# sqlp/sedumi

Hardware: AMD Instinct MI355X
Metric: IPM iters/sec (ADA' form+factor+solve) (higher is better)
Workload: dtype f64; 1 GPU; control07.mat: examples/control07.mat (BASELINE.json configs[1]), m=666, nnz(At)=107940, nnz(ADA')=443556, nnz(L)=222111; unit = getada1+2+3, blkchol, 4x(fwblkslv,./d,bwblkslv); parallelism=single GPU

## Files before the change

include/sedumi_hip.h:

```cpp
#ifndef SEDUMI_HIP_H
#define SEDUMI_HIP_H

#include <stdint.h>

#ifdef __cplusplus
extern "C" {
#endif

typedef int64_t sdm_int;

const char *sdm_last_error(void);
const char *sdm_backend(void);
int sdm_device_count(void);
int sdm_set_device(int dev);

typedef struct {
  double canceltol;
  double maxu;
  double abstol;
} sdm_cholpars;

typedef struct {
  sdm_int lpN;
  sdm_int lorN;
// ... 156 lines not shown

int sdm_plan_set_dense(sdm_plan *p, sdm_int nden, const sdm_int *LADjc, const sdm_int *LADir, const sdm_int *dzjc,
                       const sdm_int *dzir, const sdm_int *colperm, const sdm_int *first);
int sdm_plan_deninfac(sdm_plan *p, const double *smult, double maxuden, int *host_fallback);
int sdm_plan_lden(sdm_plan *p, sdm_int *betajc, double *beta, double *pv, sdm_int *pivperm, sdm_int *npivperm,
                  sdm_int *dopiv, double *Ld);

int sdm_plan_set_growth_max(sdm_plan *p, double growth_max);
int sdm_plan_set_refinement(sdm_plan *p, int mode, double refine_max);
int sdm_plan_set_one_launch_fronts(sdm_plan *p, int on);
int sdm_plan_set_tile_workgroups(sdm_plan *p, int n);
int sdm_plan_set_one_launch_inverse(sdm_plan *p, int on);
int sdm_plan_set_solve_width(sdm_plan *p, sdm_int width);
int sdm_plan_get_solve_width(sdm_plan *p, sdm_int *width);
int sdm_plan_solve_stats(sdm_plan *p, sdm_int *nblocks, sdm_int *nbad, double *max_growth);

int sdm_plan_set_active_supernodes(sdm_plan *p, const int *active, sdm_int nsuper);
int sdm_plan_front_layout(sdm_plan *p, sdm_int *nlevels, sdm_int *level, sdm_int *foff, sdm_int *fsize, sdm_int *woff, sdm_int *ms, sdm_int *first, sdm_int *ns);
int sdm_plan_blkchol_begin(sdm_plan *p, const sdm_cholpars *pars, int use_absd);
int sdm_plan_blkchol_levels(sdm_plan *p, sdm_int l0, sdm_int l1, int extend_only);
int sdm_plan_blkchol_end(sdm_plan *p);
int sdm_plan_solve_levels(sdm_plan *p, int what, sdm_int l0, sdm_int l1);

int sdm_plan_blkchol_panels(sdm_plan *p, sdm_int l0, sdm_int l1, sdm_int pan0, sdm_int pan1, int world, int rank, int blk);
int sdm_plan_panel_record(sdm_plan *p, sdm_int panel, int unpack, sdm_int *front_offset, sdm_int *front_nelem);

int sdm_mexcache_getada1(sdm_int m, const sdm_int *ADAjc, const sdm_int *ADAir, sdm_int N, const sdm_int *Ajc, const sdm_int *Air,
                         const double *Apr, const sdm_int *Ajc2, const sdm_int *perm, sdm_int lpN, const double *dl, sdm_int lorN,
                         const double *ddet, const sdm_int *qblkstart, double *ADApr, double token_in, double *token_out);
int sdm_mexcache_getada2(sdm_int m, const sdm_int *ADAjc, const sdm_int *ADAir, const double *ADApr_in, double *ADApr, sdm_int lorN,
// ... 37 lines not shown
```

sedumi_amd/capi.py:

```python
from __future__ import annotations

import ctypes as C
import os

import numpy as np

_HERE = os.path.dirname(os.path.abspath(__file__))
DEFAULT_LIB = os.path.join(_HERE, "lib", "libsedumi_hip.so")
_lib = None
_lib_path = None

I64P = C.POINTER(C.c_int64)
F64P = C.POINTER(C.c_double)


class SdmError(RuntimeError):
    pass


class CholPars(C.Structure):
    _fields_ = [("canceltol", C.c_double), ("maxu", C.c_double), ("abstol", C.c_double)]


class CgPars(C.Structure):
# ... 24 lines not shown
                       "(hipcc, gfx950).  sedumi_amd has no CPU fallback.")
    L = C.CDLL(path)
    L.sdm_last_error.restype = C.c_char_p
    L.sdm_backend.restype = C.c_char_p
    L.sdm_plan_create.restype = C.c_void_p
    L.sdm_plan_create.argtypes = [C.c_int, C.c_void_p]
    L.sdm_plan_destroy.argtypes = [C.c_void_p]
    L.sdm_plan_devptr.restype = C.c_void_p
    L.sdm_plan_devptr.argtypes = [C.c_void_p, C.c_char_p, I64P]
    for name in ("sdm_plan_sync", "sdm_plan_getada", "sdm_plan_getdatq", "sdm_plan_fwsolve", "sdm_plan_bwsolve", "sdm_plan_ldlsolve"):
        getattr(L, name).argtypes = [C.c_void_p]
    L.sdm_plan_blkchol.argtypes = [C.c_void_p, C.POINTER(CholPars), C.c_int]
    L.sdm_plan_upload.argtypes = [C.c_void_p, C.c_char_p, F64P, C.c_int64]
    L.sdm_plan_download.argtypes = [C.c_void_p, C.c_char_p, F64P, C.c_int64]
    L.sdm_plan_wrappcg.argtypes = [C.c_void_p, C.POINTER(CgPars), C.c_double, C.c_int, C.c_int, I64P, I64P]
    L.sdm_plan_timer_begin.argtypes = [C.c_void_p, C.c_int]
    L.sdm_plan_timer_end.argtypes = [C.c_void_p, C.c_int]
    L.sdm_plan_timer_ms.argtypes = [C.c_void_p, C.c_int, C.POINTER(C.c_float)]
    _lib = L
    return L


def check(rc):
    if rc:
        raise SdmError(lib().sdm_last_error().decode())


def backend():
    return lib().sdm_backend().decode()

# ... 27 lines not shown
```

sedumi_amd/csrc/sdm_ada.hip:

```cpp
#include "sdm_plan.h"
#include <algorithm>
#include <cmath>
#include <cstdlib>

namespace sdm {

__global__ void k_dsqr(double *dsqr, const int *code, const double *dl, const double *ddet, int nlq) {
  int r = blockIdx.x * blockDim.x + threadIdx.x;
  if (r < nlq) { int c = code[r]; dsqr[r] = c == -1 ? dl[r] : (c >= 0 ? ddet[c] : -ddet[-2 - c]); }
}
__global__ void k_fill(double *x, double v, int64_t n) {
  int64_t t = (int64_t)blockIdx.x * blockDim.x + threadIdx.x;
  int64_t stride = (int64_t)gridDim.x * blockDim.x;
  for (; t < n; t += stride) x[t] = v;
}

constexpr int SPDOT_CAP = 2048;
template <int LPE>
__global__ void __launch_bounds__(256)
k_ada_spdot(double *ada, const int64_t *ADAjc, const int *ADAir, const int64_t *Mbeg, const int64_t *Mend,
            const int *Mir, const double *Mpr, const double *wgt, const int *invperm, int accumulate, int jbase, int cap) {
  SDM_DYN_SMEM(smem);
  double *jv = (double *)smem;
  int *jr = (int *)(jv + cap);
// ... 654 lines not shown
        }
        const double term = Apr[p] * (zv / 2);
        acc += term; aabs += fabs(term);
      }
    const double base = base_zero ? 0.0 : ada[e];
    ada[e] = base + acc;
    if (i == j) absd[j] = jhas ? base + aabs : 0.0;
  }
}

template <int JB>
__global__ void __launch_bounds__(64 * ELL_WAVES)
k_psd_stage2_ell(double *ada, double *absd, const int64_t *ADAjc, const int *ADAir, const int64_t *Ajc,
                 const int64_t *Ajc_psd, const double *Apr, const int *Ablk, const int *Aupos,
                 const int64_t *c_taskptr, const int *t_blk, const int *t_ulen, const int64_t *t_zoff, const double *zbuf,
                 const int64_t *uoff, const int *g_row, const int *g_len, const int64_t *g_off, const double *g_val,
                 const int *g_pos, int ngroups, const int *invperm, int zmax, int m, int jbase, int jend, const int *ell_pos, const int *ell_order,
                 const int *Azpos, const int *t_zdst, int base_zero, const long long *cd64, const int *cd32) {
  SDM_DYN_SMEM(smem);
  double *zl = (double *)smem;
  __shared__ double absred[JB][ELL_WAVES];
  __shared__ double part[JB][ELL_WAVES][64];
  const int j0 = jbase + blockIdx.x * JB;
  const int tid = threadIdx.x, bs = blockDim.x;
  const int wave = tid >> 6, lane = tid & 63, nw = bs >> 6;
  int gq[JB], gstart = 0;
  if (ell_order) {
    gstart = ngroups;
#pragma unroll
    for (int q = 0; q < JB; q++) { gq[q] = min(j0 + q, jend - 1) >> 6; gstart = min(gstart, gq[q]); }
  } else {
#pragma unroll
    for (int q = 0; q < JB; q++) gq[q] = 0;
  }
  constexpr int SEG_MAX = 4 * JB;
  __shared__ long long sg_src[SEG_MAX];
  __shared__ int sg_dst[SEG_MAX], sg_cum[SEG_MAX + 1];
  __shared__ long long tb_s[JB], te_s[JB], ab_s[JB], ae_s[JB];
  __shared__ int jc_s[JB];
  for (int k = tid; k < zmax * JB; k += bs) zl[k] = 0.0;
  if (tid < SEG_MAX) {
    const int q = tid >> 2, sgi = tid & 3;
    const int x = min(j0 + q, jend - 1);
    const bool in = j0 + q < jend;
    const int nt = cd32[16 * x + 1];
    if (sgi == 0) {
      jc_s[q] = cd32[16 * x];
      const long long tb = cd64[8 * x];
      tb_s[q] = in ? tb : 0; te_s[q] = in ? tb + nt : 0;
      ab_s[q] = in ? cd64[8 * x + 1] : 0; ae_s[q] = in ? cd64[8 * x + 2] : 0;
    }
    const bool live = in && sgi < nt;
    sg_src[tid] = cd64[8 * x + 3 + sgi]; sg_dst[tid] = q * zmax + cd32[16 * x + 2 + sgi]; sg_cum[tid + 1] = live ? cd32[16 * x + 6 + sgi] : 0;
  }
  if (tid == 0) sg_cum[0] = 0;
  const int g0 = gstart + (int)blockIdx.y;
  int i0 = -1, len0 = 0;
  long long off0 = 0;
  if (g0 < ngroups) { i0 = g_row[g0 * 64 + lane]; len0 = g_len[g0]; off0 = g_off[g0]; }
  __syncthreads();
#define ELLCOL(x) (jc_s[(x) - j0 < JB ? (x) - j0 : JB - 1])
  bool jhas[JB], own[JB], owns = false;
  bool inl = true;
#pragma unroll
  for (int q = 0; q < JB; q++) {
    jhas[q] = te_s[q] > tb_s[q];
    inl = inl && te_s[q] - tb_s[q] <= 4;
    const int grp = ell_order ? gq[q] : (ell_pos[min(j0 + q, jend - 1)] >> 6);
    own[q] = j0 + q < jend && (int)blockIdx.y == (grp - gstart) % (int)gridDim.y;
    owns = owns || own[q];
  }
  if (inl) {
    if (tid == 0) for (int x = 0; x < SEG_MAX; x++) sg_cum[x + 1] += sg_cum[x];
    __syncthreads();
    const int ntot = sg_cum[SEG_MAX];
    for (int base = 0; base < ntot; base += 12 * bs) {
      double v[12]; int dd[12];
#pragma unroll
      for (int x = 0; x < 12; x++) {
        const int idx = base + x * bs + tid;
        dd[x] = -1; v[x] = 0.0;
        if (idx < ntot) {
          int sgi = 0;
          while (idx >= sg_cum[sgi + 1]) sgi++;
// ... 30 lines not shown
    __syncthreads();
    if (tid < JB && own[tid]) {
      const int j = ELLCOL(j0 + tid);
      double basev = 0.0;
      int64_t lo = ADAjc[j], hi = ADAjc[j + 1];
      const int64_t ce = hi;
      if (ce - lo == m) lo += j;
      else while (lo < hi) { const int64_t mid = (lo + hi) >> 1; if (ADAir[mid] < j) lo = mid + 1; else hi = mid; }
      if (lo < ce && ADAir[lo] == j) basev = ada[lo];
      double a = 0.0;
      for (int w = 0; w < nw; w++) a += absred[tid][w];
      absd[j] = jhas[tid] ? basev + a : 0.0;
    }
    __syncthreads();
  }
  for (int g = g0; g < ngroups; g += gridDim.y) {
    const bool first = g == g0;
    const int i = first ? i0 : g_row[g * 64 + lane];
    const int len = first ? len0 : g_len[g];
    const int64_t goff = first ? off0 : g_off[g];
    const double *gv = g_val + goff * 64 + lane;
    const int *gp = g_pos + goff * 64 + lane;
    double acc[JB];
#pragma unroll
    for (int q = 0; q < JB; q++) acc[q] = 0.0;
    int t = wave;
    for (; t + 7 * nw < len; t += 8 * nw) {
      double v[8]; int pos[8];
#pragma unroll
      for (int x = 0; x < 8; x++) { const int64_t tt = t + x * nw; v[x] = gv[tt * 64]; pos[x] = gp[tt * 64]; }
#pragma unroll
      for (int x = 0; x < 8; x++)
#pragma unroll
        for (int q = 0; q < JB; q++) acc[q] += v[x] * zl[(size_t)q * zmax + pos[x]];
    }
// ... 104 lines not shown
  if (A.q_dense) {
    SDM_HIP_CHECK(hipMemsetAsync(A.Q_d.p, 0, (size_t)A.lorN * (size_t)A.m * sizeof(double), P->stream));
    SDM_KLAUNCH(P, k_q_densify, dim3((unsigned)((A.nnzQ + 255) / 256)), dim3(256), 0, A.Q_d.p, A.qpr.p, A.q_dst.p, (int64_t)A.nnzQ);
    launch_gram(P, ada, A.Q_d.p, nullptr, A.lorN, nullptr, 0, d_invperm, accumulate, nullptr);
  } else launch_spdot(P, ada, A.d_Qjc.p, A.d_Qjc.p + 1, A.d_Qir.p, A.qpr.p, nullptr, A.q_maxcol, d_invperm, accumulate);
}
bool ada_lq_q(sdm_plan *P, double *ada) {
  AdaPlan &A = P->ada;
  if (!(A.lq_dense && A.q_dense && A.q_src.n && A.col0 == 0 && A.col1 == A.m && A.lorN > 0 && A.nnzQ > 0)) return false;
  const int64_t nq = (int64_t)A.lorN * (int)A.m, nprep = std::max<int64_t>(nq, A.nlq);
  SDM_KLAUNCH(P, k_lq_q_prep, dim3((unsigned)((nprep + 255) / 256)), dim3(256), 0, A.dsqr.p, A.dsqr_code.p, A.dl.p, A.ddet.p, (int)A.nlq,
              A.Q_d.p, A.qpr.p, A.q_src.p, nq);
  launch_gram(P, ada, A.Alq_d.p, A.dsqr.p, A.nlq, A.Q_d.p, A.lorN, nullptr, false, A.sdpN == 0 ? P->absd.p : nullptr);
  return true;
}
static void symmetrize_in_place(sdm_plan *P, double *ada) {
  AdaPlan &A = P->ada;
  SDM_KLAUNCH(P, k_symmetrize, dim3((int)A.m), dim3(128), 0, A.symtmp.p, ada, A.d_ADAjc.p, A.d_ADAir.p, A.d_ADAT.p, (int)A.m);
  SDM_HIP_CHECK(hipMemcpyAsync(ada, A.symtmp.p, A.symtmp.n * sizeof(double), hipMemcpyDeviceToDevice, P->stream));
}
static Stage1Tab stage1_tab(const AdaPlan &A) {
  Stage1Tab T;
  T.t_n = A.t_n.p; T.t_nslot = A.t_nslot.p; T.t_ulen = A.t_ulen.p; T.t_herm = A.t_herm.p; T.s_col = A.s_col.p;
  T.u_pos = A.u_pos.p; T.u_rc = A.u_rc.p; T.Air = A.d_Air.p; T.t_slotptr = A.t_slotptr.p; T.t_udoff = A.t_udoff.p; T.t_uoff = A.t_uoff.p;
  T.t_zoff = A.t_zoff.p; T.t_end = A.t_end.p; T.s_nzptr = A.s_nzptr.p; T.Apr = A.d_Apr.p; T.t_blk = A.t_blk.p;
  T.psd_start = A.d_psd_start.p;
  return T;
}
static Stage2Ride stage2_ride(sdm_plan *P, double *ada, const int *d_invperm) {
  const AdaPlan &A = P->ada;
  Stage2Ride R2 = {};
  R2.ada = ada; R2.absd = P->absd.p; R2.ADAjc = A.d_ADAjc.p; R2.Ajc = A.d_Ajc.p; R2.Ajc_psd = A.d_Ajc_psd.p; R2.ADAir = A.d_ADAir.p;
  R2.Ablk = A.d_Ablk.p; R2.Aupos = A.d_Aupos.p; R2.t_col = A.t_col.p; R2.invperm = d_invperm; R2.Apr = A.d_Apr.p;
  return R2;
}
template <int JB>
static void launch_stage2_ell(sdm_plan *P, double *ada, const int *d_invperm, int ncols, int jbase, bool sym, int gsplit, bool cleared) {
  AdaPlan &A = P->ada;
  const size_t lds = (size_t)JB * (size_t)A.zmax * sizeof(double);
#ifndef SDM_EMU
  if (lds > 48 * 1024) SDM_HIP_CHECK(hipFuncSetAttribute((const void *)k_psd_stage2_ell<JB>, hipFuncAttributeMaxDynamicSharedMemorySize, (int)lds));
#endif
  SDM_KLAUNCH_AS(P, P->stream, JB == 4 ? "k_psd_stage2_ell<4>" : JB == 2 ? "k_psd_stage2_ell<2>" : "k_psd_stage2_ell<1>", k_psd_stage2_ell<JB>,
                 dim3((ncols + JB - 1) / JB, gsplit), dim3(64 * ELL_WAVES), lds, ada, P->absd.p, A.d_ADAjc.p, A.d_ADAir.p,
                 A.d_Ajc.p, A.d_Ajc_psd.p, A.d_Apr.p, A.d_Ablk.p, A.d_Aupos.p, A.c_taskptr.p, A.t_blk.p, A.t_ulen.p,
                 A.t_zoff.p, A.zbuf.p, A.d_uoff.p, A.g_row.p, A.g_len.p, A.g_off.p, A.g_val.p, A.g_bu.p, A.ell_ng, d_invperm,
                 (int)A.zmax, (int)A.m, jbase, jbase + ncols, A.ell_pos.p, sym ? (const int *)A.ell_order.p : (const int *)nullptr,
                 A.d_Azpos.p, A.t_zdst.p, cleared ? 1 : 0,
                 sym ? (const long long *)A.cdp64.p : (const long long *)A.cdc64.p, sym ? (const int *)A.cdp32.p : (const int *)A.cdc32.p);
}
void ada_psd(sdm_plan *P, double *ada, const int *d_invperm, bool sym_input, bool absd_done) {
  AdaPlan &A = P->ada;
  const int m = (int)A.m;
  if (A.sdpN == 0 || sym_input || A.col1 <= A.col0) ada_zero_flush(P);
  if (A.sdpN == 0) {
    if (sym_input) symmetrize_in_place(P, ada);
    if (!absd_done) SDM_KLAUNCH(P, k_diag, dim3((m + 255) / 256), dim3(256), 0, P->absd.p, ada, A.d_ADAjc.p, A.d_ADAir.p, m);
    return;
  }
  if (A.col1 <= A.col0) return;
  const int ncols = (int)(A.col1 - A.col0), jbase = (int)A.col0;
  const int task0 = (int)A.h_taskptr[A.col0], ntask = (int)(A.h_taskptr[A.col1] - A.h_taskptr[A.col0]);
  const size_t direct_lds = (size_t)(2 * A.sdpN + 2 * S1_DIRECT_MAXNZ * A.sdpN + 2) * sizeof(int) + (size_t)(2 * A.sdpN) * sizeof(long long) +
                            (size_t)(S1_DIRECT_MAXNZ * A.sdpN) * sizeof(double);
// ... 47 lines not shown
      const bool ride = A.one_task_per_col && A.thread_per_row && !A.ell_ok && A.sdpN == A.rsdpN && A.s1_maxulen <= 6 * 512 &&
                        (int64_t)A.s1_maxulen * (int64_t)sizeof(double) <= (int64_t)ldsy;
      if (ride) {
        if (sym_input) symmetrize_in_place(P, ada);
        SDM_HIP_CHECK(hipMemsetAsync(P->absd.p + jbase, 0, (size_t)ncols * sizeof(double), P->stream));
      }
      SDM_KLAUNCH(P, k_psd_stage1, dim3((unsigned)ntask), dim3(512), lds, T, A.udsqr.p, A.zbuf.p, (int)(ldsy / sizeof(double)), task0, nzcap,
                  ride ? stage2_ride(P, ada, d_invperm) : Stage2Ride{},
                  (ntask == (int)A.ntask && A.t_order_xcd.n == (size_t)ntask) ? (const int *)A.t_order_xcd.p : (const int *)nullptr);
      if (ride) { SDM_HIP_CHECK(hipGetLastError()); return; }
    }
  }
  if (sym_input) symmetrize_in_place(P, ada);
  if (A.ell_ok) {
    const bool sym = A.ell_full && !d_invperm && jbase == 0 && ncols == m;
    const int gsplit = sym ? 3 : 1;
    const bool cleared = stage1_cleared_all && !sym_input;
    const size_t zbytes = (size_t)A.zmax * sizeof(double);
    if (4 * zbytes <= 64 * 1024 && m >= 1024) launch_stage2_ell<4>(P, ada, d_invperm, ncols, jbase, sym, gsplit, cleared);
    else if (2 * zbytes <= 64 * 1024 && m >= 512) launch_stage2_ell<2>(P, ada, d_invperm, ncols, jbase, sym, gsplit, cleared);
    else launch_stage2_ell<1>(P, ada, d_invperm, ncols, jbase, sym, gsplit, cleared);
  } else {
    const int64_t zl = (A.thread_per_row && A.zmaxj * 8 <= 64 * 1024) ? A.zmaxj : 0;
    const size_t lds = (size_t)A.sdpN * 8 + (size_t)zl * 8;
#ifndef SDM_EMU
    if (lds > 48 * 1024) SDM_HIP_CHECK(hipFuncSetAttribute((const void *)k_psd_stage2, hipFuncAttributeMaxDynamicSharedMemorySize, (int)lds));
#endif
    SDM_KLAUNCH(P, k_psd_stage2, dim3(ncols), dim3(256), lds, ada, P->absd.p, A.d_ADAjc.p, A.d_ADAir.p, A.d_Ajc.p,
               A.d_Ajc_psd.p, A.d_Apr.p, A.d_Ablk.p, A.d_Aupos.p, A.c_taskptr.p, A.t_blk.p, A.t_zoff.p, A.c_zlen.p, A.zbuf.p,
               d_invperm, (int)A.sdpN, A.thread_per_row ? 1 : 0, jbase, (int)zl);
  }
  SDM_HIP_CHECK(hipGetLastError());
}

}

// ... 8 lines not shown
```

sedumi_amd/csrc/sdm_ada_build.hip:

```cpp
#include "sdm_plan.h"
#include <algorithm>

namespace sdm {
namespace {

struct AdaIn {
  sdm_int m; const sdm_int *Ajc, *Air; const double *Apr; const sdm_int *Ajc_psd;
  sdm_int lpN, lorN, sdpN, rsdpN; const sdm_int *sdpNL, *qblkstart, *psd_blkstart, *Qjc, *Qir, *ADAjc, *ADAir;
  sdm_int psd_begin(sdm_int j) const { return sdpN > 0 ? Ajc_psd[j] : Ajc[j + 1]; }
};
struct PsdPatterns {
  std::vector<int> Ablk, Aupos;
  std::vector<std::vector<int>> U;
  std::vector<int64_t> uoff;
  sdm_int psdnnz = 0;
};
struct Stage1Tasks {
  std::vector<int> t_col, t_blk, t_n, t_nslot, t_ulen, t_herm, s_col, order, order_xcd;
  std::vector<int64_t> t_slotptr, t_udoff, t_uoff, t_zoff, t_end, s_nzptr, c_taskptr, c_zlen;
};

void upload_narrow(DevBuf<int> &d, const sdm_int *h, sdm_int n) { std::vector<int> v((size_t)n); for (sdm_int t = 0; t < n; t++) v[t] = (int)h[t]; d.upload(v); }

PsdPatterns psd_patterns(AdaPlan &A, const AdaIn &in) {
// ... 138 lines not shown
  std::vector<int> zp((size_t)A.nnzA, 0);
  for (sdm_int i = 0; i < m; i++) for (sdm_int t = Ajc_psd[i]; t < Ajc[i + 1]; t++) zp[(size_t)t] = (int)(pt.uoff[pt.Ablk[t]] + pt.Aupos[t]);
  std::vector<int> zd(tk.t_blk.size());
  for (size_t t = 0; t < tk.t_blk.size(); t++) zd[t] = (int)pt.uoff[tk.t_blk[t]];
  std::vector<double> gval((size_t)goff[ng] * 64, 0.0);
  std::vector<int> gbu((size_t)goff[ng] * 64, 0);
  for (int g = 0; g < ng; g++)
    for (int l = 0; l < 64; l++) {
      const int i = grow[g * 64 + l];
      if (i < 0) continue;
      for (sdm_int t = Ajc_psd[i]; t < Ajc[i + 1]; t++) {
        const size_t pos = (size_t)(goff[g] + (t - Ajc_psd[i])) * 64 + l;
        gval[pos] = in.Apr[t]; gbu[pos] = zp[(size_t)t];
      }
    }
  A.ell_ng = ng;
  A.g_row.upload(grow); A.g_len.upload(glen); A.g_off.upload(goff); A.g_val.upload(gval); A.g_bu.upload(gbu);
  { std::vector<int> pos((size_t)m); for (sdm_int p = 0; p < m; p++) pos[(size_t)order[p]] = (int)p; A.ell_pos.upload(pos); }
  A.ell_order.upload(order);
  A.ell_full = (in.ADAjc[m] == (sdm_int)m * m);
  A.d_uoff.upload(pt.uoff); A.d_Azpos.upload(zp); A.t_zdst.upload(zd);
  ell_column_records(in, tk, zd, nullptr, A.cdc64, A.cdc32);
  ell_column_records(in, tk, zd, order.data(), A.cdp64, A.cdp32);
  A.ell_ok = true;
}

std::vector<int> ada_transpose_map(const AdaIn &in) {
  const sdm_int m = in.m, *ADAjc = in.ADAjc, *ADAir = in.ADAir;
  std::vector<int> adaT((size_t)ADAjc[m], -1);
  for (sdm_int j = 0; j < m; j++)
    for (sdm_int e = ADAjc[j]; e < ADAjc[j + 1]; e++) {
      sdm_int i = ADAir[e];
      const sdm_int *b = ADAir + ADAjc[i], *en = ADAir + ADAjc[i + 1];
      const sdm_int *f = std::lower_bound(b, en, j);
      if (f != en && *f == j) adaT[e] = (int)(f - ADAir);
    }
  return adaT;
}

void lq_dense_forms(AdaPlan &A, const AdaIn &in) {
// ... 82 lines not shown
  const AdaIn in = {m, Ajc, Air, Apr, Ajc_psd, lpN, lorN, sdpN, rsdpN, sdpNL, qblkstart, psd_blkstart, Qjc, Qir, ADAjc, ADAir};
  A.N = N; A.m = m; A.nnzA = Ajc[m]; A.lpN = lpN; A.lorN = lorN; A.sdpN = sdpN; A.rsdpN = rsdpN;
  A.ic_n.release(); A.ufac.release();
  if (A.nnzA >= (sdm_int)1 << 31 || N >= (sdm_int)1 << 31) throw std::runtime_error("At too large for 32-bit row indices");
  A.nlq = sdpN > 0 ? psd_blkstart[0] : N;
  if (lorN > 0 && qblkstart[lorN] != A.nlq && sdpN > 0) throw std::runtime_error("qblkstart / psd_blkstart mismatch");
  const PsdPatterns pt = psd_patterns(A, in);
  A.thread_per_row = (m > 0 && pt.psdnnz / (double)m < 48.0);
  A.nnz_lq = A.nnzA - pt.psdnnz;
  A.nnzQ = lorN > 0 ? Qjc[m] : 0;
  A.lq_maxcol = 0; A.q_maxcol = 0;
  for (sdm_int j = 0; j < m; j++) A.lq_maxcol = std::max<int64_t>(A.lq_maxcol, in.psd_begin(j) - Ajc[j]);
  for (sdm_int j = 0; j < m && lorN > 0; j++) A.q_maxcol = std::max<int64_t>(A.q_maxcol, Qjc[j + 1] - Qjc[j]);
  const Stage1Tasks tk = stage1_tasks(A, in, pt);
  stage2_ell(A, in, pt, tk);
  upload_tables(A, in, pt, tk, ada_transpose_map(in));
  lq_dense_forms(A, in);
  P->has_ada = true;
}

}
```

sedumi_amd/csrc/sdm_capi.hip:

```cpp
#include "../../include/sedumi_hip.h"
#include "sdm_plan.h"
#include <algorithm>
#include <cstring>
#include <memory>

namespace sdm {
static thread_local std::string g_err;
void set_error(const std::string &msg) { g_err = msg; }
}
using namespace sdm;

static const char *const FACTOR_TIMEOUT = "blkchol: a workgroup timed out waiting for another one inside a factor launch";
static void check_plan_health(sdm_plan *p) {
  const int t = chol_wait_timeouts(p);
  if (t & TMO_FACTOR) throw std::runtime_error(FACTOR_TIMEOUT);
  if (t & TMO_SWEEP) throw std::runtime_error("solve: a workgroup timed out waiting for another one inside a merged sweep launch (the factor stays; the next solves run unmerged)");
}
static sdm_cholpars chol_pars(const sdm_cholpars *pars) {
  sdm_cholpars q = {1e-12, 5e2, 1e-20};
  if (pars) q = *pars;
  if (q.abstol < 0.0) q.abstol = 0.0;
  return q;
}
static void require_begun(sdm_plan *p, const char *fn) {
// ... 365 lines not shown
  SDM_CATCH
}
int sdm_plan_set_solve_width(sdm_plan *p, sdm_int width) {
  SDM_TRY
  if (width != 0 && (width < sdm::SBW_MIN || width > sdm::SBW_MAX || (width & (width - 1)) != 0))
    throw std::runtime_error("solve width must be 0 (automatic) or a power of two in 256 .. 2048");
  p->chol.sbw_req = (int)width;
  SDM_CATCH
}
int sdm_plan_get_solve_width(sdm_plan *p, sdm_int *width) {
  SDM_TRY
  if (!p->has_chol) throw std::runtime_error("sdm_plan_get_solve_width: no symbolic factor set");
  *width = p->chol.sbw;
  SDM_CATCH
}
int sdm_plan_solve_stats(sdm_plan *p, sdm_int *nblocks, sdm_int *nbad, double *max_growth) {
  SDM_TRY
  if (!p->has_chol) throw std::runtime_error("sdm_plan_solve_stats: no symbolic factor set");
  solve_stats(p, nblocks, nbad, max_growth);
  SDM_CATCH
}
int sdm_plan_pcg_init(sdm_plan *p, sdm_int nden, const sdm_int *dense_cols, const double *denseA) {
  SDM_TRY
  if (!p->has_ada) throw std::runtime_error("sdm_plan_pcg_init: no problem data set (sdm_plan_set_ada)");
  SDM_HIP_CHECK(hipSetDevice(p->device));
  pcg_set_dense(p, nden, dense_cols, denseA);
  SDM_CATCH
}
int sdm_plan_amul(sdm_plan *p, int transp) {
  SDM_TRY
// ... 420 lines not shown
```

sedumi_amd/csrc/sdm_plan.h:

```cpp
#pragma once
#include "../../include/sedumi_hip.h"
#include "sdm_rt.h"
#include <mutex>
#include <string>
#include <vector>

namespace sdm {

constexpr int NB = 64;
constexpr int TILE = 64;
constexpr int UTP = 72;
constexpr int S1_MAXN = 96;
constexpr int S1_KC = 32;
constexpr int S1_WAVES = 8;
constexpr int S1_NZ = 1536;
constexpr int s1_nzcap(int64_t maxnz) { return (int)(((maxnz + 1) & ~(int64_t)1) < S1_NZ ? ((maxnz + 1) & ~(int64_t)1) : S1_NZ); }
constexpr int s1_mfma_ldsy(int maxn) { return 2 * S1_KC * ((maxn + 15) & ~15) > maxn * (maxn | 1) ? 2 * S1_KC * ((maxn + 15) & ~15) : maxn * (maxn | 1); }
constexpr size_t s1_mfma_lds(int maxn, int64_t maxnz) { return (size_t)s1_mfma_ldsy(maxn) * sizeof(double) + (size_t)s1_nzcap(maxnz) * (sizeof(double) + sizeof(int)); }
constexpr int S1_MAXT = ((S1_MAXN / 16) * (S1_MAXN / 16) + S1_WAVES - 1) / S1_WAVES;
constexpr int S1_GEN_LDS = 74 * 1024;
constexpr int ELL_WAVES = 8;
constexpr int SOLVE_LDS_MAX = 3072;
constexpr int FUSE_MAX_TILES = 1 << 20;
constexpr int SBW_MIN = 256;
// ... 178 lines not shown
  int sweep_seq = 0;
  HostFlag noted;
};

struct FrontTab {
  const int *first, *ns, *ms, *ld;
  const int64_t *foff, *xl, *woff, *roff, *toff;
  const int *childptr, *childlist, *lindx, *relidx;
  const int64_t *soff; const int *sld, *sboff;
  const int64_t *ltoff = nullptr;
  const int *fslot = nullptr;
  int one = 0, o_s = 0, o_ns = 0, o_ms = 0, o_ld = 0, o_first = 0, o_sld = 0, o_sboff = 0;
  int64_t o_foff = 0, o_soff = 0, o_woff = 0, o_xl = 0, o_ltoff = 0;
};

struct AdaPlan {
  sdm_int N = 0, m = 0, nnzA = 0, lpN = 0, lorN = 0, sdpN = 0, rsdpN = 0;
  sdm_int nlq = 0;
  sdm_int lenud = 0, ntask = 0, zlen = 0, nnzQ = 0, nnz_lq = 0;
  int maxn = 0;
  bool thread_per_row = false;
  sdm_int col0 = 0, col1 = 0;
  double *zero_ptr = nullptr; long long zero_n = 0; bool zero_defer = false;
  std::vector<int64_t> h_taskptr;
  std::vector<sdm_int> psd_n, psd_start, psd_udoff;
  DevBuf<int64_t> d_Ajc, d_Ajc_psd, d_Qjc, d_ADAjc;
  DevBuf<int> d_Air, d_Qir, d_ADAir, d_ADAT;
  DevBuf<double> d_Apr;
  DevBuf<int> d_Ablk, d_Aupos;
  DevBuf<int> t_col, t_blk, t_n, t_nslot, t_ulen, t_herm, t_order, t_order_xcd;
// ... 30 lines not shown
  PinnedInts wp_host;
  size_t stage1_lds = 0;
  bool ell_ok = false;
  int ell_ng = 0;
  int64_t zmax = 0, zmaxj = 0;
  DevBuf<int64_t> c_zlen;
  DevBuf<int> g_row, g_len, g_bu;
  DevBuf<long long> cdc64, cdp64;
  DevBuf<int> cdc32, cdp32;
  DevBuf<int> d_Azpos, t_zdst;
  DevBuf<int> ell_pos;
  DevBuf<int> ell_order;
  bool ell_full = false;
  DevBuf<int64_t> g_off, d_uoff;
  DevBuf<double> g_val;
};

}

namespace sdm {
struct KProf {
  bool enabled = false;
  struct Rec { const char *name; hipEvent_t a, b; };
  std::vector<Rec> recs;
  std::vector<hipEvent_t> pool;
  hipEvent_t get() {
    if (!pool.empty()) { hipEvent_t e = pool.back(); pool.pop_back(); return e; }
    hipEvent_t e; SDM_HIP_CHECK(hipEventCreate(&e)); return e;
  }
};
// ... 143 lines not shown
                      const double *Apr, const sdm_int *Ajc2, sdm_int lpN, sdm_int lorN, const sdm_int *qblkstart);
void gw_run_getada1(sdm_plan *p, const int *d_invperm, const double *dl, const double *ddet);
void gw_build_getada2(sdm_plan *p, sdm_int m, const sdm_int *ADAjc, const sdm_int *ADAir, sdm_int lorN, const sdm_int *Qjc, const sdm_int *Qir);
void gw_run_getada2(sdm_plan *p, const int *d_invperm, const double *Qpr);
void gw_build_getada3(sdm_plan *p, sdm_int m, const sdm_int *ADAjc, const sdm_int *ADAir, sdm_int N, const sdm_int *Ajc, const sdm_int *Air,
                      const double *Apr, const sdm_int *Ajc1, const sdm_cone *K, const sdm_int *psd_blkstart);
void gw_run_getada3(sdm_plan *p, const double *udsqr, bool input_is_zero);
bool gw_getada1_is_zero(sdm_plan *p);
void gw_build_getada(sdm_plan *p, sdm_int m, const sdm_int *ADAjc, const sdm_int *ADAir, const sdm_int *Ajc, const sdm_int *Air, const double *Apr,
                     sdm_int lpN, sdm_int lorN, const sdm_int *qblkstart, const sdm_int *Qjc, const sdm_int *Qir);
void gw_run_getada(sdm_plan *p, const double *dl, const double *ddet, const double *Qpr);
void gw_download(sdm_plan *p, double *ADApr, double *absd);
void ada_build(sdm_plan *P, sdm_int N, sdm_int m, const sdm_int *Ajc, const sdm_int *Air, const double *Apr, const sdm_int *Ajc_psd, sdm_int lpN,
               sdm_int lorN, sdm_int sdpN, sdm_int rsdpN, const sdm_int *sdpNL, const sdm_int *qblkstart, const sdm_int *psd_blkstart,
               const sdm_int *Qjc, const sdm_int *Qir, const sdm_int *ADAjc, const sdm_int *ADAir);
void ada_zero_flush(sdm_plan *P);
void ada_lq(sdm_plan *P, double *ada, const int *d_invperm, bool accumulate);
void ada_q(sdm_plan *P, double *ada, const int *d_invperm, bool accumulate);
void ada_psd(sdm_plan *P, double *ada, const int *d_invperm, bool sym_input, bool absd_done = false);
bool ada_lq_q(sdm_plan *P, double *ada);
void ada_datq(sdm_plan *P);
void psd_invcholfac(hipStream_t st, const double *u, double *y, const int *perm, const std::vector<int> &ns, int rsdpN,
                    DevBuf<int> &d_n, DevBuf<int64_t> &d_off, DevBuf<int> &d_poff, bool tables_ready);
}
```

sedumi_amd/plan.py:

```python
from __future__ import annotations

import ctypes as C

import numpy as np
import scipy.sparse as sp

from . import capi
from .capi import SdmError, check, f64, i64, pf, pi


def _cholpars(pars):
    cp = capi.CholPars(1e-12, 5e5, 1e-20)
    if pars:
        cp.canceltol = float(pars.get("canceltol", cp.canceltol))
        cp.maxu = float(pars.get("maxu", cp.maxu))
        cp.abstol = max(float(pars.get("abstol", cp.abstol)), 0.0)
    return cp


class Plan:
    def __init__(self, device=0, stream=None):
        self._lib = capi.lib()
        self._p = self._lib.sdm_plan_create(int(device), C.c_void_p(stream) if stream else None)
        if not self._p:
# ... 158 lines not shown

    def set_tile_workgroups(self, n):
        check(self._lib.sdm_plan_set_tile_workgroups(C.c_void_p(self._p), C.c_int(int(n))))

    def set_one_launch_inverse(self, on):
        check(self._lib.sdm_plan_set_one_launch_inverse(C.c_void_p(self._p), C.c_int(1 if on else 0)))

    def set_solve_width(self, width):
        check(self._lib.sdm_plan_set_solve_width(C.c_void_p(self._p), C.c_int64(int(width))))

    def solve_width(self):
        w = C.c_int64(0)
        check(self._lib.sdm_plan_get_solve_width(C.c_void_p(self._p), C.byref(w)))
        return w.value

    def solve_stats(self):
        nb, bad, g = C.c_int64(0), C.c_int64(0), C.c_double(0.0)
        check(self._lib.sdm_plan_solve_stats(C.c_void_p(self._p), C.byref(nb), C.byref(bad), C.byref(g)))
        return nb.value, bad.value, g.value

    def getdatq(self):
        check(self._lib.sdm_plan_getdatq(C.c_void_p(self._p)))

    def getada_cols(self, j0, j1):
        check(self._lib.sdm_plan_getada_cols(C.c_void_p(self._p), C.c_int64(int(j0)), C.c_int64(int(j1))))

    def copy(self, name, tensor, offset, nelem, to_plan):
        if tensor.dtype.itemsize != 8 or not tensor.is_contiguous() or tensor.numel() < nelem:
            raise SdmError("copy: need a contiguous float64 tensor with at least nelem elements")
        if not tensor.is_cuda and capi.backend() != "emu":
# ... 117 lines not shown
```

Baseline: 2815 IPM iters/s.

## Deal PSD stage-2 ELL group work to blocks with a cost-balanced precomputed work list

Replaces the fixed 2D grid (column sets × a split of 3 over ELL row groups, strided) in the PSD stage-2 ELL kernel with a 1D grid driven by host-built work records. Each record names a column set, a list of groups, and an owner mask. The default balanced mode sizes the list to the occupancy-derived slot count and bin-packs groups by estimated cost, sorting records heaviest first. The aim is to remove load imbalance and idle blocks in ADA' formation. In exchange it adds a per-entry list indirection, a host-side planning step, and extra device tables.

```diff
diff --git a/include/sedumi_hip.h b/include/sedumi_hip.h
--- a/include/sedumi_hip.h
+++ b/include/sedumi_hip.h
@@ -194,6 +194,13 @@
 int sdm_plan_set_solve_width(sdm_plan *p, sdm_int width);
 int sdm_plan_get_solve_width(sdm_plan *p, sdm_int *width);
 int sdm_plan_solve_stats(sdm_plan *p, sdm_int *nblocks, sdm_int *nbad, double *max_growth);
+
+#define SDM_DEAL_BALANCED 0
+#define SDM_DEAL_UNIFORM 1
+#define SDM_DEAL_UNIFORM_PACKED 2
+int sdm_plan_set_stage2_dealing(sdm_plan *p, int mode, sdm_int n);
+int sdm_plan_get_stage2_dealing(sdm_plan *p, int which, sdm_int *info, sdm_int *rec, sdm_int rec_cap, sdm_int *ent, sdm_int ent_cap,
+                                sdm_int *glen, sdm_int glen_cap);
 
 int sdm_plan_set_active_supernodes(sdm_plan *p, const int *active, sdm_int nsuper);
 int sdm_plan_front_layout(sdm_plan *p, sdm_int *nlevels, sdm_int *level, sdm_int *foff, sdm_int *fsize, sdm_int *woff, sdm_int *ms, sdm_int *first, sdm_int *ns);
diff --git a/sedumi_amd/capi.py b/sedumi_amd/capi.py
--- a/sedumi_amd/capi.py
+++ b/sedumi_amd/capi.py
@@ -62,6 +62,8 @@
     L.sdm_plan_upload.argtypes = [C.c_void_p, C.c_char_p, F64P, C.c_int64]
     L.sdm_plan_download.argtypes = [C.c_void_p, C.c_char_p, F64P, C.c_int64]
     L.sdm_plan_wrappcg.argtypes = [C.c_void_p, C.POINTER(CgPars), C.c_double, C.c_int, C.c_int, I64P, I64P]
+    L.sdm_plan_set_stage2_dealing.argtypes = [C.c_void_p, C.c_int, C.c_int64]
+    L.sdm_plan_get_stage2_dealing.argtypes = [C.c_void_p, C.c_int, I64P, I64P, C.c_int64, I64P, C.c_int64, I64P, C.c_int64]
     L.sdm_plan_timer_begin.argtypes = [C.c_void_p, C.c_int]
     L.sdm_plan_timer_end.argtypes = [C.c_void_p, C.c_int]
     L.sdm_plan_timer_ms.argtypes = [C.c_void_p, C.c_int, C.POINTER(C.c_float)]
diff --git a/sedumi_amd/csrc/sdm_ada.hip b/sedumi_amd/csrc/sdm_ada.hip
--- a/sedumi_amd/csrc/sdm_ada.hip
+++ b/sedumi_amd/csrc/sdm_ada.hip
@@ -692,21 +692,23 @@
 k_psd_stage2_ell(double *ada, double *absd, const int64_t *ADAjc, const int *ADAir, const int64_t *Ajc,
                  const int64_t *Ajc_psd, const double *Apr, const int *Ablk, const int *Aupos,
                  const int64_t *c_taskptr, const int *t_blk, const int *t_ulen, const int64_t *t_zoff, const double *zbuf,
-                 const int64_t *uoff, const int *g_row, const int *g_len, const int64_t *g_off, const double *g_val,
-                 const int *g_pos, int ngroups, const int *invperm, int zmax, int m, int jbase, int jend, const int *ell_pos, const int *ell_order,
-                 const int *Azpos, const int *t_zdst, int base_zero, const long long *cd64, const int *cd32) {
+                 const int64_t *uoff, const int *g_row, const double *g_val,
+                 const int *g_pos, const int *invperm, int zmax, int m, int jbase, int jend, const int *ell_order,
+                 const int *Azpos, const int *t_zdst, int base_zero, const long long *cd64, const int *cd32,
+                 const S2Quad *__restrict__ s2rec, const S2Quad *__restrict__ s2ent) {
   SDM_DYN_SMEM(smem);
   double *zl = (double *)smem;
   __shared__ double absred[JB][ELL_WAVES];
   __shared__ double part[JB][ELL_WAVES][64];
-  const int j0 = jbase + blockIdx.x * JB;
+  const S2Quad rec = s2rec[2 * blockIdx.x];
+  S2Quad ent = s2rec[2 * blockIdx.x + 1];
+  const int j0 = jbase + rec.x * JB;
   const int tid = threadIdx.x, bs = blockDim.x;
   const int wave = tid >> 6, lane = tid & 63, nw = bs >> 6;
-  int gq[JB], gstart = 0;
+  int gq[JB];
   if (ell_order) {
-    gstart = ngroups;
-#pragma unroll
-    for (int q = 0; q < JB; q++) { gq[q] = min(j0 + q, jend - 1) >> 6; gstart = min(gstart, gq[q]); }
+#pragma unroll
+    for (int q = 0; q < JB; q++) gq[q] = min(j0 + q, jend - 1) >> 6;
   } else {
 #pragma unroll
     for (int q = 0; q < JB; q++) gq[q] = 0;
@@ -732,10 +734,9 @@
     sg_src[tid] = cd64[8 * x + 3 + sgi]; sg_dst[tid] = q * zmax + cd32[16 * x + 2 + sgi]; sg_cum[tid + 1] = live ? cd32[16 * x + 6 + sgi] : 0;
   }
   if (tid == 0) sg_cum[0] = 0;
-  const int g0 = gstart + (int)blockIdx.y;
-  int i0 = -1, len0 = 0;
-  long long off0 = 0;
-  if (g0 < ngroups) { i0 = g_row[g0 * 64 + lane]; len0 = g_len[g0]; off0 = g_off[g0]; }
+  const int necnt = rec.z;
+  int i0 = -1;
+  if (necnt > 0) i0 = g_row[ent.x * 64 + lane];
   __syncthreads();
 #define ELLCOL(x) (jc_s[(x) - j0 < JB ? (x) - j0 : JB - 1])
   bool jhas[JB], own[JB], owns = false;
@@ -744,8 +745,7 @@
   for (int q = 0; q < JB; q++) {
     jhas[q] = te_s[q] > tb_s[q];
     inl = inl && te_s[q] - tb_s[q] <= 4;
-    const int grp = ell_order ? gq[q] : (ell_pos[min(j0 + q, jend - 1)] >> 6);
-    own[q] = j0 + q < jend && (int)blockIdx.y == (grp - gstart) % (int)gridDim.y;
+    own[q] = j0 + q < jend && ((rec.w >> q) & 1);
     owns = owns || own[q];
   }
   if (inl) {
@@ -806,11 +806,11 @@
     }
     __syncthreads();
   }
-  for (int g = g0; g < ngroups; g += gridDim.y) {
-    const bool first = g == g0;
-    const int i = first ? i0 : g_row[g * 64 + lane];
-    const int len = first ? len0 : g_len[g];
-    const int64_t goff = first ? off0 : g_off[g];
+  for (int k = 0; k < necnt; k++) {
+    const int g = ent.x, len = ent.y;
+    const int64_t goff = ent.z;
+    const int i = k == 0 ? i0 : g_row[g * 64 + lane];
+    if (k + 1 < necnt) ent = s2ent[rec.y + k + 1];
     const double *gv = g_val + goff * 64 + lane;
     const int *gp = g_pos + goff * 64 + lane;
     double acc[JB];
@@ -945,6 +945,32 @@
   launch_gram(P, ada, A.Alq_d.p, A.dsqr.p, A.nlq, A.Q_d.p, A.lorN, nullptr, false, A.sdpN == 0 ? P->absd.p : nullptr);
   return true;
 }
+int stage2_ell_jb(const AdaPlan &A) {
+  const size_t zbytes = (size_t)A.zmax * sizeof(double);
+  return (4 * zbytes <= 64 * 1024 && A.m >= 1024) ? 4 : (2 * zbytes <= 64 * 1024 && A.m >= 512) ? 2 : 1;
+}
+template <int JB>
+static int stage2_ell_per_cu(size_t lds) {
+  int per_cu = 0;
+#ifndef SDM_EMU
+  if (lds > 48 * 1024) SDM_HIP_CHECK(hipFuncSetAttribute((const void *)k_psd_stage2_ell<JB>, hipFuncAttributeMaxDynamicSharedMemorySize, (int)lds));
+  SDM_HIP_CHECK(hipOccupancyMaxActiveBlocksPerMultiprocessor(&per_cu, (const void *)k_psd_stage2_ell<JB>, 64 * ELL_WAVES, lds));
+#endif
+  return per_cu;
+}
+int stage2_ell_slots(sdm_plan *P, int jb, int *per_cu_out) {
+#ifdef SDM_EMU
+  if (per_cu_out) *per_cu_out = S2_EMU_SLOTS / 256;
+  return S2_EMU_SLOTS;
+#else
+  const size_t lds = (size_t)jb * (size_t)P->ada.zmax * sizeof(double);
+  const int per_cu = jb == 4 ? stage2_ell_per_cu<4>(lds) : jb == 2 ? stage2_ell_per_cu<2>(lds) : stage2_ell_per_cu<1>(lds);
+  int ncu = 0;
+  SDM_HIP_CHECK(hipDeviceGetAttribute(&ncu, hipDeviceAttributeMultiprocessorCount, P->device));
+  if (per_cu_out) *per_cu_out = per_cu;
+  return std::max(1, per_cu * ncu);
+#endif
+}
 static void symmetrize_in_place(sdm_plan *P, double *ada) {
   AdaPlan &A = P->ada;
   SDM_KLAUNCH(P, k_symmetrize, dim3((int)A.m), dim3(128), 0, A.symtmp.p, ada, A.d_ADAjc.p, A.d_ADAir.p, A.d_ADAT.p, (int)A.m);
@@ -966,19 +992,23 @@
   return R2;
 }
 template <int JB>
-static void launch_stage2_ell(sdm_plan *P, double *ada, const int *d_invperm, int ncols, int jbase, bool sym, int gsplit, bool cleared) {
+static void launch_stage2_ell(sdm_plan *P, double *ada, const int *d_invperm, int ncols, int jbase, bool sym, bool cleared) {
   AdaPlan &A = P->ada;
+  if (A.deal_jb != JB) throw std::runtime_error("k_psd_stage2_ell: no work list for this launch");
+  const int nrec = sym ? A.deal_sym.nrec() : (ncols + JB - 1) / JB;
+  if (!sym && nrec > A.deal_all.nrec()) throw std::runtime_error("k_psd_stage2_ell: work list shorter than the launch");
   const size_t lds = (size_t)JB * (size_t)A.zmax * sizeof(double);
 #ifndef SDM_EMU
   if (lds > 48 * 1024) SDM_HIP_CHECK(hipFuncSetAttribute((const void *)k_psd_stage2_ell<JB>, hipFuncAttributeMaxDynamicSharedMemorySize, (int)lds));
 #endif
   SDM_KLAUNCH_AS(P, P->stream, JB == 4 ? "k_psd_stage2_ell<4>" : JB == 2 ? "k_psd_stage2_ell<2>" : "k_psd_stage2_ell<1>", k_psd_stage2_ell<JB>,
-                 dim3((ncols + JB - 1) / JB, gsplit), dim3(64 * ELL_WAVES), lds, ada, P->absd.p, A.d_ADAjc.p, A.d_ADAir.p,
+                 dim3(nrec), dim3(64 * ELL_WAVES), lds, ada, P->absd.p, A.d_ADAjc.p, A.d_ADAir.p,
                  A.d_Ajc.p, A.d_Ajc_psd.p, A.d_Apr.p, A.d_Ablk.p, A.d_Aupos.p, A.c_taskptr.p, A.t_blk.p, A.t_ulen.p,
-                 A.t_zoff.p, A.zbuf.p, A.d_uoff.p, A.g_row.p, A.g_len.p, A.g_off.p, A.g_val.p, A.g_bu.p, A.ell_ng, d_invperm,
-                 (int)A.zmax, (int)A.m, jbase, jbase + ncols, A.ell_pos.p, sym ? (const int *)A.ell_order.p : (const int *)nullptr,
+                 A.t_zoff.p, A.zbuf.p, A.d_uoff.p, A.g_row.p, A.g_val.p, A.g_bu.p, d_invperm,
+                 (int)A.zmax, (int)A.m, jbase, jbase + ncols, sym ? (const int *)A.ell_order.p : (const int *)nullptr,
                  A.d_Azpos.p, A.t_zdst.p, cleared ? 1 : 0,
-                 sym ? (const long long *)A.cdp64.p : (const long long *)A.cdc64.p, sym ? (const int *)A.cdp32.p : (const int *)A.cdc32.p);
+                 sym ? (const long long *)A.cdp64.p : (const long long *)A.cdc64.p, sym ? (const int *)A.cdp32.p : (const int *)A.cdc32.p,
+                 (const S2Quad *)(sym ? A.s2rec_sym.p : A.s2rec_all.p), (const S2Quad *)(sym ? A.s2ent_sym.p : A.s2ent_all.p));
 }
 void ada_psd(sdm_plan *P, double *ada, const int *d_invperm, bool sym_input, bool absd_done) {
   AdaPlan &A = P->ada;
@@ -1056,12 +1086,12 @@
   if (sym_input) symmetrize_in_place(P, ada);
   if (A.ell_ok) {
     const bool sym = A.ell_full && !d_invperm && jbase == 0 && ncols == m;
-    const int gsplit = sym ? 3 : 1;
     const bool cleared = stage1_cleared_all && !sym_input;
-    const size_t zbytes = (size_t)A.zmax * sizeof(double);
-    if (4 * zbytes <= 64 * 1024 && m >= 1024) launch_stage2_ell<4>(P, ada, d_invperm, ncols, jbase, sym, gsplit, cleared);
-    else if (2 * zbytes <= 64 * 1024 && m >= 512) launch_stage2_ell<2>(P, ada, d_invperm, ncols, jbase, sym, gsplit, cleared);
-    else launch_stage2_ell<1>(P, ada, d_invperm, ncols, jbase, sym, gsplit, cleared);
+    switch (stage2_ell_jb(A)) {
+      case 4: launch_stage2_ell<4>(P, ada, d_invperm, ncols, jbase, sym, cleared); break;
+      case 2: launch_stage2_ell<2>(P, ada, d_invperm, ncols, jbase, sym, cleared); break;
+      default: launch_stage2_ell<1>(P, ada, d_invperm, ncols, jbase, sym, cleared);
+    }
   } else {
     const int64_t zl = (A.thread_per_row && A.zmaxj * 8 <= 64 * 1024) ? A.zmaxj : 0;
     const size_t lds = (size_t)A.sdpN * 8 + (size_t)zl * 8;
diff --git a/sedumi_amd/csrc/sdm_ada_build.hip b/sedumi_amd/csrc/sdm_ada_build.hip
--- a/sedumi_amd/csrc/sdm_ada_build.hip
+++ b/sedumi_amd/csrc/sdm_ada_build.hip
@@ -176,7 +176,8 @@
         gval[pos] = in.Apr[t]; gbu[pos] = zp[(size_t)t];
       }
     }
-  A.ell_ng = ng;
+  if (goff[ng] > INT32_MAX) throw std::runtime_error("ELL copy of the PSD nonzeros too long for 32-bit offsets");
+  A.ell_ng = ng; A.h_glen = glen;
   A.g_row.upload(grow); A.g_len.upload(glen); A.g_off.upload(goff); A.g_val.upload(gval); A.g_bu.upload(gbu);
   { std::vector<int> pos((size_t)m); for (sdm_int p = 0; p < m; p++) pos[(size_t)order[p]] = (int)p; A.ell_pos.upload(pos); }
   A.ell_order.upload(order);
@@ -186,6 +187,95 @@
   ell_column_records(in, tk, zd, order.data(), A.cdp64, A.cdp32);
   A.ell_ok = true;
 }
+
+}
+
+Stage2Deal stage2_deal(const std::vector<int> &g_len, int m, int jb, int slots, int mode, int n, bool sym) {
+  const int ng = (int)g_len.size(), nsets = (m + jb - 1) / jb;
+  std::vector<int> gc((size_t)ng), goff((size_t)ng + 1, 0);
+  for (int g = 0; g < ng; g++) { gc[g] = stage2_group_cost(g_len[g]); goff[g + 1] = goff[g] + g_len[g]; }
+  typedef std::vector<std::vector<int>> Lists;
+  auto cost = [&](const std::vector<int> &l) { int c = S2_PROLOGUE_TRIPS; for (int g : l) c += gc[g]; return c; };
+  auto whole = [&](int own) { Lists r(1); for (int g = own; g < ng; g++) r[0].push_back(g); return r; };
+  auto single = [&](int own) { Lists r; for (int g = own; g < ng; g++) r.push_back(std::vector<int>(1, g)); return r; };
+  auto uniform = [&](int own, bool empties) {
+    Lists r;
+    for (int y = 0; y < n; y++) {
+      std::vector<int> l;
+      for (int g = own + y; g < ng; g += n) l.push_back(g);
+      if (!l.empty() || empties || y == 0) r.push_back(l);
+    }
+    return r;
+  };
+  auto packed = [&](int own, int L) {
+    std::vector<int> gs;
+    for (int g = own; g < ng; g++) gs.push_back(g);
+    std::stable_sort(gs.begin(), gs.end(), [&](int a, int b) { return gc[a] > gc[b]; });
+    Lists r; std::vector<int> load;
+    for (int g : gs) {
+      size_t b = 0;
+      while (b < r.size() && load[b] + gc[g] > L) b++;
+      if (b == r.size()) { r.emplace_back(); load.push_back(S2_PROLOGUE_TRIPS); }
+      r[b].push_back(g); load[b] += gc[g];
+    }
+    return r;
+  };
+  std::vector<int> nown((size_t)std::max(ng, 1), 0);
+  for (int x = 0; x < nsets; x++) nown[sym ? std::min((x * jb) >> 6, ng - 1) : 0]++;
+  std::vector<Lists> by_own((size_t)std::max(ng, 1));
+  const int nowns = sym ? ng : 1;
+  if (!sym) by_own[0] = whole(0);
+  else if (mode == SDM_DEAL_UNIFORM || mode == SDM_DEAL_UNIFORM_PACKED) for (int o = 0; o < nowns; o++) by_own[o] = uniform(o, mode == SDM_DEAL_UNIFORM);
+  else {
+    int64_t pairs = 0;
+    for (int o = 0; o < nowns; o++) pairs += (int64_t)nown[o] * (ng - o);
+    if (nsets > slots) for (int o = 0; o < nowns; o++) by_own[o] = whole(o);
+    else if (pairs <= slots) for (int o = 0; o < nowns; o++) by_own[o] = single(o);
+    else {
+      int L = S2_PROLOGUE_TRIPS + (ng > 0 ? *std::max_element(gc.begin(), gc.end()) : 0);
+      for (;; L++) {
+        int64_t tot = 0;
+        for (int o = 0; o < nowns; o++) { by_own[o] = packed(o, L); tot += (int64_t)nown[o] * (int64_t)by_own[o].size(); }
+        if (tot <= slots) break;
+      }
+    }
+  }
+  struct R { int set, own, li, cost; };
+  std::vector<R> recs;
+  for (int x = 0; x < nsets; x++) {
+    const int o = sym ? std::min((x * jb) >> 6, ng - 1) : 0;
+    for (size_t li = 0; li < by_own[o].size(); li++) recs.push_back({x, o, (int)li, cost(by_own[o][li])});
+  }
+  std::stable_sort(recs.begin(), recs.end(), [](const R &a, const R &b) { return a.cost > b.cost; });
+  Stage2Deal D;
+  auto entry = [&](std::vector<int> &v, int g) { v.push_back(g); v.push_back(g_len[g]); v.push_back(goff[g]); v.push_back(0); };
+  if (!sym) for (int g = 0; g < ng; g++) entry(D.ent, g);
+  for (const R &r : recs) {
+    const std::vector<int> &l = by_own[r.own][r.li];
+    const bool owner = !sym || std::find(l.begin(), l.end(), r.own) != l.end();
+    D.rec.push_back(r.set); D.rec.push_back(sym ? (int)(D.ent.size() / 4) : 0); D.rec.push_back((int)l.size()); D.rec.push_back(owner ? (1 << jb) - 1 : 0);
+    if (l.empty()) D.rec.insert(D.rec.end(), 4, 0); else entry(D.rec, l[0]);
+    if (sym) for (int g : l) entry(D.ent, g);
+    D.cost.push_back(r.cost);
+  }
+  return D;
+}
+
+void stage2_dealing(sdm_plan *P) {
+  AdaPlan &A = P->ada;
+  A.deal_sym = Stage2Deal(); A.deal_all = Stage2Deal(); A.deal_jb = 0; A.deal_slots = 0;
+  if (!A.ell_ok) { A.s2rec_sym.release(); A.s2ent_sym.release(); A.s2rec_all.release(); A.s2ent_all.release(); return; }
+  A.deal_jb = stage2_ell_jb(A);
+  A.deal_slots = (A.deal_mode == SDM_DEAL_BALANCED && A.deal_n > 0) ? A.deal_n : stage2_ell_slots(P, A.deal_jb);
+  A.deal_all = stage2_deal(A.h_glen, (int)A.m, A.deal_jb, A.deal_slots, A.deal_mode, A.deal_n, false);
+  A.s2rec_all.upload(A.deal_all.rec); A.s2ent_all.upload(A.deal_all.ent);
+  if (A.ell_full) {
+    A.deal_sym = stage2_deal(A.h_glen, (int)A.m, A.deal_jb, A.deal_slots, A.deal_mode, A.deal_n, true);
+    A.s2rec_sym.upload(A.deal_sym.rec); A.s2ent_sym.upload(A.deal_sym.ent);
+  } else { A.s2rec_sym.release(); A.s2ent_sym.release(); }
+}
+
+namespace {
 
 std::vector<int> ada_transpose_map(const AdaIn &in) {
   const sdm_int m = in.m, *ADAjc = in.ADAjc, *ADAir = in.ADAir;
@@ -298,6 +388,7 @@
   for (sdm_int j = 0; j < m && lorN > 0; j++) A.q_maxcol = std::max<int64_t>(A.q_maxcol, Qjc[j + 1] - Qjc[j]);
   const Stage1Tasks tk = stage1_tasks(A, in, pt);
   stage2_ell(A, in, pt, tk);
+  stage2_dealing(P);
   upload_tables(A, in, pt, tk, ada_transpose_map(in));
   lq_dense_forms(A, in);
   P->has_ada = true;
diff --git a/sedumi_amd/csrc/sdm_capi.hip b/sedumi_amd/csrc/sdm_capi.hip
--- a/sedumi_amd/csrc/sdm_capi.hip
+++ b/sedumi_amd/csrc/sdm_capi.hip
@@ -403,6 +403,40 @@
   *width = p->chol.sbw;
   SDM_CATCH
 }
+int sdm_plan_set_stage2_dealing(sdm_plan *p, int mode, sdm_int n) {
+  SDM_TRY
+  if (mode != SDM_DEAL_BALANCED && mode != SDM_DEAL_UNIFORM && mode != SDM_DEAL_UNIFORM_PACKED) throw std::runtime_error("sdm_plan_set_stage2_dealing: unknown mode");
+  if (n < 0 || n > (1 << 24) || (mode != SDM_DEAL_BALANCED && n < 1)) throw std::runtime_error("sdm_plan_set_stage2_dealing: n out of range");
+  if (p->capturing) throw std::runtime_error("sdm_plan_set_stage2_dealing: not during a graph capture");
+  p->ada.deal_mode = mode; p->ada.deal_n = (int)n;
+  if (p->has_ada) {
+    SDM_HIP_CHECK(hipSetDevice(p->device));
+    SDM_HIP_CHECK(hipStreamSynchronize(p->stream));
+    stage2_dealing(p);
+  }
+  SDM_CATCH
+}
+int sdm_plan_get_stage2_dealing(sdm_plan *p, int which, sdm_int *info, sdm_int *rec, sdm_int rec_cap, sdm_int *ent, sdm_int ent_cap,
+                                sdm_int *glen, sdm_int glen_cap) {
+  SDM_TRY
+  if (!p->has_ada) throw std::runtime_error("sdm_plan_get_stage2_dealing: no problem data set (sdm_plan_set_ada)");
+  const AdaPlan &A = p->ada;
+  const bool sym = which == 0 && A.ell_full && A.deal_jb > 0;
+  const Stage2Deal &D = sym ? A.deal_sym : A.deal_all;
+  const sdm_int nrec = D.nrec(), nent = (sdm_int)(D.ent.size() / 4), ng = A.deal_jb > 0 ? (sdm_int)A.h_glen.size() : 0;
+  if (info) {
+    const sdm_int v[8] = {A.deal_jb, ng, A.deal_slots, A.deal_mode, A.deal_n, nrec, nent, sym ? 1 : 0};
+    std::copy(v, v + 8, info);
+  }
+  if (rec)
+    for (sdm_int r = 0; r < std::min(nrec, rec_cap); r++) {
+      for (int x = 0; x < 4; x++) rec[5 * r + x] = D.rec[8 * r + x];
+      rec[5 * r + 4] = D.cost[r];
+    }
+  if (ent) for (sdm_int e = 0; e < std::min(nent, ent_cap); e++) ent[e] = D.ent[4 * e];
+  if (glen) for (sdm_int g = 0; g < std::min(ng, glen_cap); g++) glen[g] = A.h_glen[g];
+  SDM_CATCH
+}
 int sdm_plan_solve_stats(sdm_plan *p, sdm_int *nblocks, sdm_int *nbad, double *max_growth) {
   SDM_TRY
   if (!p->has_chol) throw std::runtime_error("sdm_plan_solve_stats: no symbolic factor set");
diff --git a/sedumi_amd/csrc/sdm_plan.h b/sedumi_amd/csrc/sdm_plan.h
--- a/sedumi_amd/csrc/sdm_plan.h
+++ b/sedumi_amd/csrc/sdm_plan.h
@@ -216,6 +216,16 @@
   int64_t o_foff = 0, o_soff = 0, o_woff = 0, o_xl = 0, o_ltoff = 0;
 };
 
+constexpr int S2_PROLOGUE_TRIPS = 5;
+constexpr int S2_EMU_SLOTS = 768;
+struct alignas(16) S2Quad { int x, y, z, w; };
+struct Stage2Deal {
+  std::vector<int> rec, ent, cost;
+  int nrec() const { return (int)cost.size(); }
+};
+inline int stage2_group_cost(int len) { return (len + 8 * ELL_WAVES - 1) / (8 * ELL_WAVES); }
+Stage2Deal stage2_deal(const std::vector<int> &g_len, int m, int jb, int slots, int mode, int n, bool sym);
+
 struct AdaPlan {
   sdm_int N = 0, m = 0, nnzA = 0, lpN = 0, lorN = 0, sdpN = 0, rsdpN = 0;
   sdm_int nlq = 0;
@@ -276,6 +286,11 @@
   bool ell_full = false;
   DevBuf<int64_t> g_off, d_uoff;
   DevBuf<double> g_val;
+  std::vector<int> h_glen;
+  int deal_mode = SDM_DEAL_BALANCED, deal_n = 0;
+  int deal_jb = 0, deal_slots = 0;
+  Stage2Deal deal_sym, deal_all;
+  DevBuf<int> s2rec_sym, s2ent_sym, s2rec_all, s2ent_all;
 };
 
 }
@@ -449,6 +464,9 @@
 void ada_build(sdm_plan *P, sdm_int N, sdm_int m, const sdm_int *Ajc, const sdm_int *Air, const double *Apr, const sdm_int *Ajc_psd, sdm_int lpN,
                sdm_int lorN, sdm_int sdpN, sdm_int rsdpN, const sdm_int *sdpNL, const sdm_int *qblkstart, const sdm_int *psd_blkstart,
                const sdm_int *Qjc, const sdm_int *Qir, const sdm_int *ADAjc, const sdm_int *ADAir);
+void stage2_dealing(sdm_plan *P);
+int stage2_ell_jb(const AdaPlan &A);
+int stage2_ell_slots(sdm_plan *P, int jb, int *per_cu = nullptr);
 void ada_zero_flush(sdm_plan *P);
 void ada_lq(sdm_plan *P, double *ada, const int *d_invperm, bool accumulate);
 void ada_q(sdm_plan *P, double *ada, const int *d_invperm, bool accumulate);
diff --git a/sedumi_amd/plan.py b/sedumi_amd/plan.py
--- a/sedumi_amd/plan.py
+++ b/sedumi_amd/plan.py
@@ -196,6 +196,25 @@
         check(self._lib.sdm_plan_get_solve_width(C.c_void_p(self._p), C.byref(w)))
         return w.value
 
+    DEAL = {"balanced": 0, "uniform": 1, "uniform_packed": 2}
+
+    def set_stage2_dealing(self, mode="balanced", n=0):
+        check(self._lib.sdm_plan_set_stage2_dealing(C.c_void_p(self._p), C.c_int(self.DEAL[mode]), C.c_int64(int(n))))
+
+    def stage2_dealing(self, which=0):
+        info = np.zeros(8, dtype=np.int64)
+        none = (None, C.c_int64(0))
+        check(self._lib.sdm_plan_get_stage2_dealing(C.c_void_p(self._p), C.c_int(which), pi(info), *none, *none, *none))
+        if info[0] == 0:
+            return None
+        rec, ent, glen = np.zeros(5 * info[5], dtype=np.int64), np.zeros(max(info[6], 1), dtype=np.int64), np.zeros(info[1], dtype=np.int64)
+        check(self._lib.sdm_plan_get_stage2_dealing(C.c_void_p(self._p), C.c_int(which), pi(info), pi(rec), C.c_int64(info[5]), pi(ent), C.c_int64(info[6]),
+                                                    pi(glen), C.c_int64(info[1])))
+        rec = rec.reshape(-1, 5)
+        return {"jb": int(info[0]), "slots": int(info[2]), "mode": {v: k for k, v in self.DEAL.items()}[int(info[3])], "n": int(info[4]),
+                "symmetric": bool(info[7]), "glen": glen.tolist(),
+                "records": [(int(s), [int(g) for g in ent[o:o + c]], int(w), int(k)) for s, o, c, w, k in rec]}
+
     def solve_stats(self):
         nb, bad, g = C.c_int64(0), C.c_int64(0), C.c_double(0.0)
         check(self._lib.sdm_plan_solve_stats(C.c_void_p(self._p), C.byref(nb), C.byref(bad), C.byref(g)))
```

Result: no change. 2834 IPM iters/s, median of 6 (+0.7%).
